# OpenDrift/opendrift

Hardware: AMD Instinct MI355X
Metric: particle-steps/sec (RK4, 3D interp) (higher is better)
Workload: dtype f64; 1 GPU; C3: OceanDrift 3D, synthetic ROMS-shaped z-level grid 1024x1024x12 (u,v,w,K), RK4 + vertical_mixing(60 s) + vertical_advection; particles_per_gpu=10000000, particles_total=10000000, stage_math=fast, spin_up_steps=200, block_every=0, inputs=resident in HBM, parallelism=particle-sharded x1, field block broadcast once per time level

## Files before the change

### include/odrift.h

```cpp
#ifndef ODRIFT_H
#define ODRIFT_H
#include <stdint.h>

#ifdef __cplusplus
extern "C" {
#endif

typedef struct odr_ctx odr_ctx;
typedef struct odr_particles odr_particles;

typedef enum {
  ODR_OK = 0,
  ODR_ERR_INVALID = -1,
  ODR_ERR_HIP = -2,
  ODR_ERR_CAPACITY = -3,
  ODR_ERR_STATE = -4
} odr_status;

enum {
  ODR_VAR_X_SEA_WATER_VELOCITY = 0,
  ODR_VAR_Y_SEA_WATER_VELOCITY = 1,
  ODR_VAR_X_WIND = 2,
  ODR_VAR_Y_WIND = 3,
  ODR_VAR_UPWARD_SEA_WATER_VELOCITY = 4,
// ... 262 lines not shown
int odr_scan_status(odr_ctx *ctx, odr_particles *p, int64_t *n_kept, uint64_t *status_flags);
int odr_scan_status_begin(odr_ctx *ctx, odr_particles *p);
int odr_scan_status_end(odr_ctx *ctx, odr_particles *p, int64_t *n_kept, uint64_t *status_flags);
int odr_ctx_guard_next_vmix(odr_ctx *ctx, int on);
int odr_compact_apply(odr_ctx *ctx, odr_particles *p, int64_t *n_active);
int odr_sort_particles(odr_ctx *ctx, odr_particles *p, int32_t source_id);
int odr_sort_particles_ex(odr_ctx *ctx, odr_particles *p, int32_t source_id, int keep_environment);
int odr_particles_tile_stats(odr_ctx *ctx, odr_particles *p, uint64_t *out4);
int odr_particles_step_layout_stats(odr_ctx *ctx, odr_particles *p, uint64_t *out2);
int odr_particles_step_onlevel_stats(odr_ctx *ctx, odr_particles *p, uint64_t *out1);
int odr_particles_vmix_layout_stats(odr_ctx *ctx, odr_particles *p, uint64_t *out3);
int odr_particles_vmix_kplane_stats(odr_ctx *ctx, odr_particles *p, uint64_t *out2);
int odr_particles_vmix_window_stats(odr_ctx *ctx, odr_particles *p, uint64_t *out3);
int odr_particles_vmix_skip_stats(odr_ctx *ctx, odr_particles *p, uint64_t *out2);
int odr_particles_vmix_dense_stats(odr_ctx *ctx, odr_particles *p, uint64_t *out2);
int odr_reduce_scalars(odr_ctx *ctx, odr_particles *p, double wind_drift_depth, double *out16);
int odr_ctx_set_step_reduce(odr_ctx *ctx, int on, double wind_drift_depth, int relative_wind);
int odr_reduce_local(odr_ctx *ctx, odr_particles *p, double wind_drift_depth, int relative_wind, double *out16);
int odr_reduce_install(odr_ctx *ctx, odr_particles *p, const double *in16);
int odr_reduce_unpin(odr_ctx *ctx);
int odr_reduce_cached(odr_ctx *ctx, odr_particles *p, double *out16, int32_t *state);

int odr_ctx_set_position_class(odr_ctx *ctx, int f32);
int odr_source_set_coordinate_dtype(odr_ctx *ctx, int32_t source_id, int x_is_float32, int y_is_float32);

#define ODR_COMM_ID_BYTES 256
int odr_device_count(int32_t *n);
int odr_comm_unique_id(uint8_t *id );
int odr_comm_init(odr_ctx *ctx, const uint8_t *id, int32_t rank, int32_t nranks);
int odr_comm_info(int32_t *rank, int32_t *nranks, uint64_t *id_hash, int32_t *rccl_version, uint64_t *collectives);
// ... 116 lines not shown
```

### opendrift_amd/_abi.py

```python
import ctypes as C
import os

HERE = os.path.dirname(os.path.abspath(__file__))
LIB_PATH = os.environ.get('ODR_LIB') or os.path.join(HERE, 'libodrift_hip.so')

NVAR = 26
VARIABLES = {
    'x_sea_water_velocity': 0, 'y_sea_water_velocity': 1, 'x_wind': 2, 'y_wind': 3,
    'upward_sea_water_velocity': 4, 'ocean_vertical_diffusivity': 5,
    'sea_surface_wave_stokes_drift_x_velocity': 6, 'sea_surface_wave_stokes_drift_y_velocity': 7,
    'land_binary_mask': 8, 'sea_floor_depth_below_sea_level': 9, 'sea_surface_height': 10,
    'horizontal_diffusivity': 11, 'sea_surface_wave_significant_height': 12,
    'sea_surface_wave_period_at_variance_spectral_density_maximum': 13,
    'ocean_mixed_layer_thickness': 14,
    'sea_water_temperature': 15, 'sea_water_salinity': 16,
    'sea_ice_area_fraction': 17, 'sea_ice_x_velocity': 18, 'sea_ice_y_velocity': 19,
    'sea_surface_swell_wave_to_direction': 20,
    'sea_surface_swell_wave_peak_period_from_variance_spectral_density': 21,
    'sea_surface_swell_wave_significant_height': 22, 'sea_surface_wind_wave_to_direction': 23,
    'sea_surface_wind_wave_mean_period': 24, 'sea_surface_wind_wave_significant_height': 25,
}
VARIABLE_NAMES = {v: k for k, v in VARIABLES.items()}
PROJ_LATLONG, PROJ_STERE_EQUIT_SPHERE, PROJ_STERE_POLAR = 0, 1, 2
PROJ_MERC, PROJ_LCC = 4, 5
# ... 168 lines not shown
    'odr_scan_status': [_vp, _vp, _i64p, _P(C.c_uint64)],
    'odr_scan_status_begin': [_vp, _vp],
    'odr_scan_status_end': [_vp, _vp, _i64p, _P(C.c_uint64)],
    'odr_ctx_guard_next_vmix': [_vp, C.c_int],
    'odr_compact_apply': [_vp, _vp, _i64p],
    'odr_sort_particles': [_vp, _vp, C.c_int32],
    'odr_sort_particles_ex': [_vp, _vp, C.c_int32, C.c_int],
    'odr_particles_tile_stats': [_vp, _vp, _P(C.c_uint64)],
    'odr_particles_step_layout_stats': [_vp, _vp, _P(C.c_uint64)],
    'odr_particles_step_onlevel_stats': [_vp, _vp, _P(C.c_uint64)],
    'odr_particles_vmix_layout_stats': [_vp, _vp, _P(C.c_uint64)],
    'odr_particles_vmix_kplane_stats': [_vp, _vp, _P(C.c_uint64)],
    'odr_particles_vmix_window_stats': [_vp, _vp, _P(C.c_uint64)],
    'odr_particles_vmix_skip_stats': [_vp, _vp, _P(C.c_uint64)],
    'odr_particles_vmix_dense_stats': [_vp, _vp, _P(C.c_uint64)],
    'odr_reduce_scalars': [_vp, _vp, C.c_double, _dp],
    'odr_ctx_set_step_reduce': [_vp, C.c_int, C.c_double, C.c_int],
    'odr_reduce_local': [_vp, _vp, C.c_double, C.c_int, _dp],
    'odr_reduce_install': [_vp, _vp, _dp],
    'odr_reduce_unpin': [_vp],
    'odr_reduce_cached': [_vp, _vp, _dp, _ip],
    'odr_timer_begin': [_vp],
    'odr_timer_end': [_vp, _fp],
    'odr_sgrid_create': [_vp, C.c_int32, C.c_int32, C.c_int32, _dp, _dp, C.c_double, _dp, _dp, C.c_int32, _P(_vp)],
    'odr_sgrid_destroy': [_vp, _vp],
    'odr_sgrid_download_zrho': [_vp, _vp, _dp],
    'odr_sgrid_zslice': [_vp, _vp, _vp, C.c_int, C.c_int, C.c_int32, _dp, C.c_int32, _P(_vp), _dp],
    'odr_history_create': [_vp, C.c_int64, C.c_int32, C.c_int32, _ip, _P(_vp)],
    'odr_history_destroy': [_vp, _vp],
    'odr_history_set_id_base': [_vp, _vp, C.c_int64],
# ... 90 lines not shown
```

### opendrift_amd/csrc/odr_host.h

```cpp
#pragma once
#include <hip/hip_runtime.h>

#include <algorithm>
#include <cmath>
#include <cstdarg>
#include <cstdio>
#include <cstdlib>
#include <cstring>
#include <initializer_list>
#include <string>
#include <vector>

#include "../../include/odrift.h"
#include "odr_kernels.hip.h"

using namespace odr;

#include <chrono>
struct SlowSpan {
  const char *what;
  std::chrono::steady_clock::time_point t0;
  static double limit() { static const double v = getenv("ODR_SLOW_CALLS") ? atof(getenv("ODR_SLOW_CALLS")) : 0.0; return v; }
  explicit SlowSpan(const char *w) : what(w) { if (limit() > 0) t0 = std::chrono::steady_clock::now(); }
  ~SlowSpan() {
// ... 118 lines not shown
  long long scan_kept;
  float env_cval[NVAR];
  long long env_cn[NVAR];
  bool env_cok[NVAR];
  bool external;
  unsigned *wg_tab, *wg_list;
  unsigned long long *wg_total, *wg_stats;
  long long wg_cap, wg_grid, wg_n, wg_list_cap;
  unsigned long long wg_launches;
  unsigned long long step_launches[3];
  unsigned long long vmix_launches[3];
  unsigned long long vmix_kplane[2];
  unsigned long long vmix_window[2];
  unsigned long long vmix_tiled;
  unsigned long long vmix_dense;
  unsigned long long *vmix_redone;
  unsigned long long *vmix_mask;
  unsigned *vmix_toff, *vmix_list;
  double *z_keep;
  long long z_keep_n;
  bool z_truncated;
  int wg_sid;
  bool wg_valid;
  unsigned wg_src_gen;
};

static inline unsigned nblk(long long n) { return (unsigned)((n + BLOCK - 1) / BLOCK); }

static inline PView view(const odr_particles *p) {
  PView v;
  v.n = p->n;
  v.lon = p->d64[0]; v.lat = p->d64[1]; v.z = p->d64[2]; v.plon = p->d64[3]; v.plat = p->d64[4];
  v.slon = p->d64[5]; v.slat = p->d64[6];
// ... 187 lines not shown
```

### opendrift_amd/csrc/odr_kernels.hip.h

```cpp
#pragma once
#include <hip/hip_runtime.h>
#include <rocrand/rocrand_kernel.h>
#include "odr_field.hip.h"

namespace odr {

#ifndef ODR_BLOCK
#define ODR_BLOCK 256
#endif
constexpr int BLOCK = ODR_BLOCK;
#ifndef ODR_POLAR_WAVES
#define ODR_POLAR_WAVES 3
#endif
#ifndef ODR_POLAR_STEP_WAVES
#define ODR_POLAR_STEP_WAVES 2
#endif
#define ODR_STEP_WAVES(PROJ) ((PROJ) == PROJ_LATLONG ? ODR_LATLONG_WAVES : ((PROJ) == PROJ_EXT ? 1 : ODR_POLAR_STEP_WAVES))
#ifndef ODR_LATLONG_WAVES
#define ODR_LATLONG_WAVES 1
#endif
#define ODR_WAVES(PROJ) ((PROJ) == PROJ_LATLONG ? ODR_LATLONG_WAVES : ((PROJ) == PROJ_EXT ? 1 : ODR_POLAR_WAVES))

__device__ __forceinline__ unsigned pid_wg_of(unsigned nb) {
  const unsigned b = blockIdx.x, per = nb >> 3, rem = nb & 7u, x = b & 7u, j = b >> 3;
// ... 833 lines not shown
  int coast_action, stranded_code, seeded_code, land_slot;
  int store_previous, geo_slot_uv;
  int seafloor, depth_slot;
  float age_dt, max_age;
  int retired_code, missing_code;
  int nmiss_grp, nmiss_rest;
  int miss_grp[4], miss_rest[4];
  int main_noise;
  int ssh_slot;
  int red_on, red_rel;
  int red_hd, red_sx, red_xw, red_pad;
  double red_wdd, red_iwdd;
  double *red;
  unsigned *wcount;
  unsigned long long *sflags;
};

#ifndef ODR_PARK_WAVES
#define ODR_PARK_WAVES 4
#endif
#ifndef ODR_PARK_WAVES_FAST3D
#define ODR_PARK_WAVES_FAST3D 5
#endif
#define ODR_PARK_WAVES_OF(PROJ, IS3D, SM) (((PROJ) == PROJ_LATLONG && (IS3D) && (SM) == 1) ? ODR_PARK_WAVES_FAST3D : ODR_PARK_WAVES)
#define ODR_STEP_PARKS(SCHEME, PROJ) ((SCHEME) > 0 && ((PROJ) == PROJ_LATLONG || (PROJ) == PROJ_CURVILINEAR))
template <int SCHEME, int PROJ, bool IS3D, bool NOISE, int SM = 0, class LY = LayoutRT>
__global__ __launch_bounds__(BLOCK, ODR_STEP_PARKS(SCHEME, PROJ) ? ODR_PARK_WAVES_OF(PROJ, IS3D, SM) : ODR_STEP_WAVES(PROJ)) void k_step_grid(const DevWorld *__restrict__ W, PView p, EnvGroupDesc G,
                                                     StepDesc S, double dt, float factor, UVTime th, UVTime tf,
                                                     unsigned long long *n_hit, StageNoise N) {
  long long i = pid();
// ... 89 lines not shown
          ps0.ok = 0;
          p.env[VAR_LAND][i] = 0.0f;
        }
      }
    }
    if (S.seafloor) {
      float floorz;
      if constexpr (LY::STATIC) {
        static_assert(LY::depth_slot >= 0 && LY::ssh_slot < 0, "a static layout holds the depth and not the ssh");
        floorz = -__fadd_rn(out[LY::depth_slot], ssh0);
      } else {
        const float dep = S.depth_slot == 2 ? out[2] : (S.depth_slot == 3 ? out[3] : p.env[VAR_DEPTH][i]);
        floorz = -__fadd_rn(dep, S.ssh_slot >= 0 ? pick_slot(out, S.ssh_slot) : ssh0);
      }
      if (zz < (double)floorz) { zz = (double)floorz; p.z[i] = zz; }
    }
    if (S.age_dt != 0.0f) {
      const float a = __fadd_rn(age0, S.age_dt);
      p.age[i] = a;
      if (S.max_age > 0 && a >= S.max_age) {
        if (st == 0) p.status[i] = st = S.retired_code;
        p.moving[i] = moving = 0;
      }
    }
    const bool skip = st != 0;
    if constexpr (IS3D && SM == 1) { if (zz != z) K.valid = false; }
    if (S.store_previous) { p.plon[i] = lon; p.plat[i] = lat; }
    ODR_PT(3);
    if (!skip) {
      const DevSource &s = W->src[G.sid];
// ... 842 lines not shown
      if (esc != 0ull) {
        if (escaped) {
          long long i2 = i;
          asm volatile("" : "+v"(i2));
          const VMixState S2 = vmix_load_state(p, i2);
          vmix_col_particle<NQ, TL, typename VM::Full>(s, p, Dp, A, vadv, i, Kp, gsh, t, S2);
          if (D.redone && (t & 63) == __ffsll((long long)esc) - 1) atomicAdd(D.redone, (unsigned long long)__popcll(esc));
        }
      }
    }
  }
}

struct VMixKeep {
  unsigned long long *mask;
  unsigned *toff;
  unsigned *list;
  unsigned *hdr;
  unsigned long long *listed;
};
__global__ __launch_bounds__(BLOCK) void k_vmix_keep(PView p, VMixKeep K, const unsigned long long *guard, double dt,
                                                      double dt_mix_cfg) {
  if (guard && *guard == 0ull) return;
  constexpr int NW = BLOCK / 64;
  __shared__ unsigned cnt[NW];
  const int tid = threadIdx.x, lane = tid & 63, wave = tid >> 6;
  const long long base = (long long)blockIdx.x * VMIX_TILE;
  double z[VMIX_TILE_ROUNDS];
  float dep[VMIX_TILE_ROUNDS], ssh[VMIX_TILE_ROUNDS];
#pragma unroll
  for (int r = 0; r < VMIX_TILE_ROUNDS; ++r) {
    const long long e = base + r * BLOCK + tid, ec = e < p.n ? e : 0;
    z[r] = p.z[ec]; dep[r] = p.env[VAR_DEPTH][ec]; ssh[r] = p.env[VAR_SSH][ec];
  }
  const double sgn = dt > 0 ? 1.0 : (dt < 0 ? -1.0 : 0.0);
  const bool walks = abs((int)(dt / (dt_mix_cfg * sgn))) > 0;
  unsigned mine = 0;
#pragma unroll
  for (int r = 0; r < VMIX_TILE_ROUNDS; ++r) {
    const long long e = base + r * BLOCK + tid;
    const float Zmin = __fmul_rn(-1.f, __fadd_rn(dep[r], ssh[r]));
    const bool skip = e < p.n && z[r] == 0 && !(Zmin > 0.f);
    if (skip && walks && __double_as_longlong(z[r]) != 0ll) p.z[e] = 0.0;
    const unsigned long long keep = __ballot(e < p.n && !skip);
    if (lane == 0) K.mask[(size_t)blockIdx.x * (VMIX_TILE / 64) + r * NW + wave] = keep;
    mine += (unsigned)__popcll(keep);
  }
  if (lane == 0) cnt[wave] = mine;
  __syncthreads();
  if (tid == 0) {
    unsigned t = 0;
#pragma unroll
    for (int w = 0; w < NW; ++w) t += cnt[w];
    K.toff[blockIdx.x] = t;
  }
}
constexpr int VMIX_SCAN_ROWS = 16;
__global__ __launch_bounds__(1024) void k_vmix_keep_scan(VMixKeep K, long long ntiles, long long n,
                                                          const unsigned long long *guard, unsigned long long *skipped) {
  const int tid = threadIdx.x, lane = tid & 63, wv = tid >> 6;
  if (guard && *guard == 0ull) {
    if (tid == 0) { K.hdr[0] = 0u; K.hdr[1] = 0u; }
    return;
  }
  constexpr int G = VMIX_SCAN_ROWS;
  __shared__ unsigned wtot[G * 16];
  unsigned carry = 0;
  for (long long k0 = 0; k0 < ntiles; k0 += (long long)G * 1024) {
    unsigned v[G], x[G];
#pragma unroll
    for (int u = 0; u < G; ++u) {
      const long long k = k0 + (long long)u * 1024 + tid;
      v[u] = k < ntiles ? K.toff[k] : 0u;
    }
#pragma unroll
    for (int u = 0; u < G; ++u) {
      x[u] = v[u];
#pragma unroll
      for (int o = 1; o < 64; o <<= 1) { const unsigned y = __shfl_up(x[u], o, 64); if (lane >= o) x[u] += y; }
      if (lane == 63) wtot[u * 16 + wv] = x[u];
    }
    __syncthreads();
    if (wv == 0) {
#pragma unroll
      for (int b0 = 0; b0 < G * 16; b0 += 64) {
        const unsigned t0 = wtot[b0 + lane];
        unsigned s = t0;
#pragma unroll
        for (int o = 1; o < 64; o <<= 1) { const unsigned y = __shfl_up(s, o, 64); if (lane >= o) s += y; }
        wtot[b0 + lane] = carry + s - t0;
        carry += __shfl(s, 63, 64);
      }
    }
    __syncthreads();
#pragma unroll
    for (int u = 0; u < G; ++u) {
      const long long k = k0 + (long long)u * 1024 + tid;
      if (k < ntiles) K.toff[k] = x[u] - v[u] + wtot[u * 16 + wv];
    }
    __syncthreads();
  }
  if (tid == 0) {
    K.hdr[0] = carry;
    K.hdr[1] = (carry + (unsigned)BLOCK - 1u) / (unsigned)BLOCK;
    if (skipped && (unsigned long long)n > carry) atomicAdd(skipped, (unsigned long long)n - carry);
    if (carry) atomicAdd(K.listed, (unsigned long long)carry);
  }
}
__global__ __launch_bounds__(BLOCK) void k_vmix_keep_fill(VMixKeep K, const unsigned long long *guard) {
  if (guard && *guard == 0ull) return;
  constexpr int NW = BLOCK / 64;
  const int tid = threadIdx.x, lane = tid & 63;
  const int wave = __builtin_amdgcn_readfirstlane(tid >> 6);
  const unsigned long long *m = K.mask + (size_t)blockIdx.x * (VMIX_TILE / 64);
  unsigned run = K.toff[blockIdx.x], off[VMIX_TILE_ROUNDS];
  unsigned long long keep[VMIX_TILE_ROUNDS];
#pragma unroll
  for (int g = 0; g < VMIX_TILE / 64; ++g) {
    const unsigned long long mg = m[g];
    if ((g % NW) == wave) { off[g / NW] = run; keep[g / NW] = mg; }
    run += (unsigned)__popcll(mg);
  }
  const unsigned long long below = (1ull << lane) - 1ull;
  const unsigned first = (unsigned)blockIdx.x * (unsigned)VMIX_TILE;
#pragma unroll
  for (int r = 0; r < VMIX_TILE_ROUNDS; ++r)
    if ((keep[r] >> lane) & 1ull) K.list[off[r] + (unsigned)__popcll(keep[r] & below)] = first + (unsigned)(r * BLOCK + tid);
}
__host__ __device__ constexpr size_t vmix_dense_lds_bytes(int nq) {
  return sizeof(double) * ((size_t)(4 * nq) * BLOCK + 4 * (size_t)(4 * nq));
}
template <int NQ, bool TL, class VM>
__global__ __launch_bounds__(BLOCK, ODR_VMIX_WAVES) void k_vmix_dense(const DevWorld *__restrict__ W, PView p, VMixDesc D,
                                                      const unsigned *__restrict__ list, const unsigned *__restrict__ hdr,
                                                      double dt, double dt_mix_cfg, int mix_at_surface,
                                                      int rng_mode, const double *__restrict__ huni,
                                                      unsigned long long seed, unsigned long long step,
                                                      int vadv, int sfl) {
  static_assert(VM::STATIC, "the dense launch exists for the static configurations");
  constexpr int NL = 4 * NQ;
  extern __shared__ __attribute__((aligned(16))) char smem[];
  const int tid = threadIdx.x;
  const DevSource &s = W->src[D.sid];
  const int nzp = VM::nzp(D.nzp, NL);
  double *Kp = (double *)smem;
  double *gsh = Kp + (size_t)NL * BLOCK;
  if (D.guard && *D.guard == 0ull) return;
  const unsigned total = hdr[0], nbd = hdr[1];
  if (blockIdx.x >= nbd) return;
  const unsigned d = pid_wg_of(nbd) * BLOCK + (unsigned)tid;
  const bool valid = d < total;
  const long long i = list[valid ? d : 0u];
  if (tid < nzp) {
    gsh[tid] = s.vg_a[tid]; gsh[NL + tid] = s.vg_b[tid]; gsh[2 * NL + tid] = s.vg_c[tid];
    gsh[3 * NL + tid] = s.zmid[tid];
  }
  long long i1 = i;
  asm volatile("" : "+v"(i1));
  const VMixState S = vmix_load_state(p, i1);
  __syncthreads();
  if (!valid) return;
  VMixArgs A;
  A.dt = dt; A.dt_mix_cfg = dt_mix_cfg; A.mix_at_surface = mix_at_surface; A.rng_mode = rng_mode; A.sfl = sfl; A.pad = 0;
  A.huni = huni; A.seed = seed; A.step = step;
  const bool escaped = vmix_col_particle<NQ, TL, VM>(s, p, D, A, vadv, i, Kp, gsh, tid, S);
  if constexpr (VM::WINDOW) {
    const unsigned long long esc = __ballot(escaped);
// ... 1481 lines not shown
```

### opendrift_amd/csrc/odr_mix.hip

```cpp
#define ODR_TU_MIX 1
#include "odr_host.h"

static_assert(vmix_col_lds_bytes(3) <= 163840 / ODR_VMIX_WAVES, "k_vmix_col<3>: column, tables and offset list exceed a sixth of the LDS");
static_assert(vmix_dense_lds_bytes(3) <= 163840 / ODR_VMIX_WAVES, "k_vmix_dense<3>: column and tables exceed a sixth of the LDS");
static_assert(VMIX_TILE == 1024, "odr_particles_create sizes the keep ballots and tile counts for tiles of 1024 elements");

template <class VM>
static bool vmix_layout_matches(const DevSource &s, const VMixDesc &D, int nq, double dt, double dt_mix, int mix_at_surface,
                                int rng_mode, int sfl, int vadv) {
  const bool uz = s.vg_uniform != 0;
  const int ntimes = abs((int)(dt / (dt_mix * (dt > 0 ? 1.0 : (dt < 0 ? -1.0 : 0.0)))));
  return VM::proj_kind(s.proj.kind) == s.proj.kind && VM::lon_mode(s.lon_mode) == s.lon_mode &&
         VM::mod360_x(s.mod360_x) == s.mod360_x && VM::nzp(D.nzp, 4 * nq) == D.nzp && VM::uniform_z(uz) == uz &&
         VM::rng_mode(rng_mode) == rng_mode && VM::mix_at_surface(mix_at_surface) == mix_at_surface &&
         VM::sf_action(sfl & 255) == (sfl & 255) && VM::vadv(vadv) == vadv && VM::ntimes(ntimes) == ntimes &&
         VM::kstride(D.kstride, nq) == D.kstride;
}

int odr_vmix(odr_ctx *c, odr_particles *p, double t, double dt, double dt_mix, int mix_at_surface, int rng_mode,
             const double *huni, uint64_t step) {
  const bool guarded = c->guard_next_vmix != 0;
  c->guard_next_vmix = 0;
  const bool oil = c->oil_owner == p;
  const bool f32prof = p->profiles_f32;
  const int cut = c->vmix_levels;
  VMixDesc D;
  bool kplanes = !getenv("ODR_NO_KPLANE");
  const bool fast = !oil && !f32prof && cut <= 0 && !getenv("ODR_NO_FAST_PATH") && build_vmix_desc(c, t, D, kplanes);
  if (guarded && (rng_mode == ODR_RNG_HOST || !fast)) return 1;
  const int vadv = c->fuse_vadv;
  c->fuse_vadv = -1;
  c->oil_owner = nullptr;
  c->vmix_levels = 0;
  c->guarded_vmix = nullptr;
  p->status_epoch++;
  p->epoch++;
  REQUIRE(dt_mix > 0 && dt != 0, "bad time steps");
  if (!p->env[VAR_DEPTH]) return fail(ODR_ERR_STATE, "sea_floor_depth_below_sea_level has not been sampled");
  if (int rs = seafloor_species_slot_ok(c, p)) return rs;
  int rc = ensure_env(c, p, VAR_SSH);
  if (rc) return rc;
  if ((rc = flush_world(c))) return rc;
  if (p->n == 0) return 0;
  int nzp = 1;
  for (int k = 0; k < c->hw.nlist[VAR_KZ]; ++k) {
    const DevSource &s = c->hw.src[c->hw.list[VAR_KZ][k]];
    if (s.kind == SRC_GRID) { nzp = s.nz > 1 ? s.nz : 1; break; }
  }
  double *du = nullptr;
// ... 32 lines not shown
    const bool spec = !win && (nq == 2 || nq == 3) &&
                      vmix_layout_matches<VMixC3Rec>(c->hw.src[D.sid], D, nq, dt, dt_mix, mix_at_surface, rng_mode, c->seafloor, vadv) &&
                      !getenv("ODR_NO_VMIX_SPEC");
    const bool specp = spec && vmix_layout_matches<VMixC3>(c->hw.src[D.sid], D, nq, dt, dt_mix, mix_at_surface, rng_mode, c->seafloor, vadv);
    const bool quadwin = spec && nq == 3 && !getenv("ODR_NO_VMIX_WINDOW");
    p->vmix_launches[win ? 2 : spec ? 1 : 0]++;
    p->vmix_kplane[kplanes ? 0 : 1]++;
    if (spec && nq == 3) p->vmix_window[quadwin ? 0 : 1]++;
    D.redone = quadwin ? p->vmix_redone : nullptr;
    D.skipped = p->vmix_redone + 1;
    D.noskip = getenv("ODR_NO_VMIX_SKIP") ? 1 : 0;
    if (!win) { g = dim3((unsigned)((p->n + VMIX_TILE - 1) / VMIX_TILE)); p->vmix_tiled++; }
    const bool dense = spec && mix_at_surface == 0 && vadv != 1 && !D.noskip && !getenv("ODR_NO_VMIX_DENSE") &&
                       p->n <= 0xffffffffLL;
    VMixKeep K;
    K.mask = p->vmix_mask; K.toff = p->vmix_toff; K.list = p->vmix_list;
    K.hdr = (unsigned *)(p->vmix_redone + 3); K.listed = p->vmix_redone + 2;
    if (dense) {
      hipLaunchKernelGGL(k_vmix_keep, g, b, 0, c->stream, v, K, D.guard, dt, dt_mix);
      hipLaunchKernelGGL(k_vmix_keep_scan, dim3(1), dim3(1024), 0, c->stream, K, (long long)g.x, (long long)p->n, D.guard, D.skipped);
      hipLaunchKernelGGL(k_vmix_keep_fill, g, b, 0, c->stream, K, D.guard);
      g = dim3(nblk(p->n));
      p->vmix_dense++;
    }
#define VMIX_DENSE(NQ, VM)                                                                                        \
  do {                                                                                                            \
    const size_t l2 = vmix_dense_lds_bytes(NQ);                                                                   \
    if (tl) hipLaunchKernelGGL((k_vmix_dense<NQ, true, VM>), g, b, l2, c->stream, c->dw, v, D, K.list, K.hdr, dt, dt_mix, \
                               mix_at_surface, rng_mode, du, c->seed, st, vadv, c->seafloor);                     \
    else hipLaunchKernelGGL((k_vmix_dense<NQ, false, VM>), g, b, l2, c->stream, c->dw, v, D, K.list, K.hdr, dt, dt_mix, \
                            mix_at_surface, rng_mode, du, c->seed, st, vadv, c->seafloor);                        \
  } while (0)
#define VMIX_COL(NQ, VM)                                                                                          \
  do {                                                                                                            \
    const size_t l2 = vmix_col_lds_bytes(NQ);                                                                     \
    if (tl) hipLaunchKernelGGL((k_vmix_col<NQ, true, VM>), g, b, l2, c->stream, c->dw, v, D, dt, dt_mix,          \
// ... 60 lines not shown
  D2H(&skipped, p->vmix_redone + 1, sizeof skipped);
  HIPCHK(hipStreamSynchronize(c->stream));
  out2[0] = p->vmix_tiled; out2[1] = skipped;
  return 0;
}

int odr_particles_vmix_dense_stats(odr_ctx *c, odr_particles *p, uint64_t *out2) {
  REQUIRE(c && p && out2, "NULL argument");
  unsigned long long listed = 0;
  D2H(&listed, p->vmix_redone + 2, sizeof listed);
  HIPCHK(hipStreamSynchronize(c->stream));
  out2[0] = p->vmix_dense; out2[1] = listed;
  return 0;
}

int odr_particles_vmix_window_stats(odr_ctx *c, odr_particles *p, uint64_t *out3) {
  REQUIRE(c && p && out3, "NULL argument");
  unsigned long long redone = 0;
  D2H(&redone, p->vmix_redone, sizeof redone);
  HIPCHK(hipStreamSynchronize(c->stream));
  out3[0] = p->vmix_window[0]; out3[1] = p->vmix_window[1]; out3[2] = redone;
  return 0;
}

int odr_vmix_set_profile_levels(odr_ctx *c, int32_t n) {
  REQUIRE(n == 0 || (n >= 2 && n <= 255), "bad level count %d", n);
  c->vmix_levels = n;
  return 0;
}

// ... 176 lines not shown
```

### opendrift_amd/csrc/odr_step.hip

```cpp
#define ODR_TU_STEP 1
#include <chrono>
#include "odr_step_launch.h"

int odr_advect_set_noise(odr_ctx *c, odr_particles *p, double std_normal, double std_uniform, int rng_mode,
                         const double *host_main, const double *host_stage, int nstage, uint64_t step) {
  c->noise_owner = nullptr;
  REQUIRE(std_normal >= 0 && std_uniform >= 0, "uncertainties must not be negative");
  REQUIRE(rng_mode == ODR_RNG_DEVICE || rng_mode == ODR_RNG_HOST, "bad rng mode");
  if (!(std_normal > 0) && !(std_uniform > 0)) return 0;
  StageNoise &N = c->noise;
  memset(&N, 0, sizeof N);
  N.on = 1; N.rng_mode = rng_mode; N.std_n = std_normal; N.std_u = std_uniform;
  N.ncomp = 2 * ((std_normal > 0) + (std_uniform > 0));
  N.seed = c->seed; N.step = (unsigned long long)step;
  if (rng_mode == ODR_RNG_HOST && p->n > 0) {
    REQUIRE(nstage >= 0 && nstage <= 3 && (nstage == 0 || host_stage), "host draws of the stage calls required in ODR_RNG_HOST mode");
    const size_t per = (size_t)N.ncomp * (size_t)p->n, need = per * (size_t)(nstage + (host_main ? 1 : 0));
    if (c->noise_buf_n < need) {
      HIPCHK(hipStreamSynchronize(c->stream));
      if (c->noise_buf) HIPCHK(hipFree(c->noise_buf));
      HIPCHK(hipMalloc((void **)&c->noise_buf, sizeof(double) * need));
      c->noise_buf_n = need;
    }
    double *d = c->noise_buf;
// ... 188 lines not shown
      const int a = slot_of(vx), b = slot_of(vy);
      if (a >= 0 && b == a + 1) { out = a; return true; }
      if (a == -1 && b == -1) { out = -1; return true; }
      if (a == -2 || b == -2) { out = -2; return a < 0 && b < 0; }
      return false;
    };
    S.red_hd = slot_of(VAR_HDIFF);
    red_in_launch = pair_of(VAR_SX, VAR_SY, S.red_sx) && pair_of(VAR_XWIND, VAR_YWIND, S.red_xw) && (S.red_xw == -2 || p->f32[0]);
    if (red_in_launch) {
      S.red_on = 1; S.red_rel = c->step_reduce_rel; S.red_wdd = c->step_reduce_wdd;
      S.red_iwdd = c->step_reduce_wdd != 0 ? 1.0 / fabs(c->step_reduce_wdd) : 0.0;
      if ((rc = odr_i_red_records(c, p, &S.red))) return rc;
    }
  }
  if (count_in_launch) { S.wcount = p->wcount; S.sflags = c->counter + 2; }
  if (N.on && (scheme > 0 || main_noise)) {
    if (scheme > 0 && N.rng_mode == ODR_RNG_HOST && !N.stage) return fail(ODR_ERR_INVALID, "no host draws for the Runge-Kutta stage calls");
    if (N.sm == ODR_STAGE_FAST && scheme > 0) odr_i_step_fast_noise(c, p, G, S, scheme, t, dt, factor, N);
    else odr_i_step_noise(c, p, G, S, scheme, t, dt, factor, N);
  } else if (N.sm == ODR_STAGE_FAST && scheme > 0) odr_i_step_fast(c, p, G, S, scheme, t, dt, factor, N);
  else step_dispatch<false>(c, p, G, S, scheme, t, dt, factor, N);
  HIPCHK(hipGetLastError());
  if (red_in_launch) {
    if ((rc = odr_i_red_finish(c, p))) return rc;
    c->red_owner = p; c->red_epoch = p->epoch; c->red_wdd = c->step_reduce_wdd; c->red_rel = c->step_reduce_rel;
    c->red_extents = false; c->red_partial = true;
  }
  mark(3);
  if (count_in_launch) { p->wcount_epoch = p->status_epoch; p->wcount_n = p->n; }
  if ((rc = coast_action ? read_counter(c, n_on_land) : 0)) return rc;
// ... 15 lines not shown
```

### opendrift_amd/csrc/odr_step_launch.h

```cpp
#pragma once
#include "odr_host.h"

template <int SCHEME, bool NOISE, int SM = 0>
static void launch_advect_grid(odr_ctx *c, odr_particles *p, int sid, double t, double dt, double factor, const StageNoise &N) {
  const DevSource &s = c->hw.src[sid];
  UVTime th = uv_time(s, t + dt / 2), tf = uv_time(s, t + dt);
  int geo = s.level_slot[0];
  bool is3d = s.slot[geo].var_nz[VAR_U] > 1;
  dim3 g(nblk(p->n)), b(BLOCK);
  PView v = view(p);
  float f = (float)factor;
#define ODR_LAUNCH(PROJ, D3) hipLaunchKernelGGL((k_advect_grid<SCHEME, PROJ, D3, NOISE, SM>), g, b, 0, c->stream, c->dw, sid, geo, v, dt, f, th, tf, N)
  switch (odr_proj_template(s.proj)) {
    case PROJ_LATLONG: if (is3d) ODR_LAUNCH(PROJ_LATLONG, true); else ODR_LAUNCH(PROJ_LATLONG, false); break;
    case PROJ_STERE_POLAR: if (is3d) ODR_LAUNCH(PROJ_STERE_POLAR, true); else ODR_LAUNCH(PROJ_STERE_POLAR, false); break;
    case PROJ_CURVILINEAR: if (is3d) ODR_LAUNCH(PROJ_CURVILINEAR, true); else ODR_LAUNCH(PROJ_CURVILINEAR, false); break;
    case PROJ_EXT: if (is3d) ODR_LAUNCH(PROJ_EXT, true); else ODR_LAUNCH(PROJ_EXT, false); break;
    default: if (is3d) ODR_LAUNCH(PROJ_STERE_EQUIT_SPHERE, true); else ODR_LAUNCH(PROJ_STERE_EQUIT_SPHERE, false); break;
  }
#undef ODR_LAUNCH
}

template <bool NOISE, int SM = 0>
static bool advect_dispatch(odr_ctx *c, odr_particles *p, int scheme, double t, double dt, double factor, const StageNoise &N) {
// ... 49 lines not shown
                             double factor, const StageNoise &N) {
  const EnvGroupDesc G = env_bind_out(G0, view(p));
  const DevSource &s = c->hw.src[G.sid];
  UVTime th = uv_time(s, t + dt / 2), tf = uv_time(s, t + dt);
  S.geo_slot_uv = s.level_slot[0];
  bool is3d = s.slot[S.geo_slot_uv].var_nz[VAR_U] > 1;
  dim3 g(nblk(p->n)), b(BLOCK);
  PView v = view(p);
  float f = (float)factor;
  if constexpr (SCHEME == 2 && !NOISE && SM == 1) {
    if (odr_proj_template(s.proj) == PROJ_LATLONG && is3d && !getenv("ODR_NO_LAYOUT_SPEC")) {
      if (layout_matches<LayoutC3>(G, S)) {
        hipLaunchKernelGGL((k_step_grid<SCHEME, PROJ_LATLONG, true, NOISE, SM, LayoutC3>), g, b, 0, c->stream, c->dw, v, G, S,
                           dt, f, th, tf, c->counter, N);
        p->step_launches[1]++;
        return;
      }
      if (layout_matches_onlevel(s, G, S, t, dt, th)) {
        hipLaunchKernelGGL((k_step_grid<SCHEME, PROJ_LATLONG, true, NOISE, SM, LayoutC3L1>), g, b, 0, c->stream, c->dw, v, G, S,
                           dt, f, th, tf, c->counter, N);
        p->step_launches[0]++;
        p->step_launches[2]++;
        return;
      }
    }
  }
  p->step_launches[0]++;
#define ODR_LAUNCH(PROJ, D3) hipLaunchKernelGGL((k_step_grid<SCHEME, PROJ, D3, NOISE, SM>), g, b, 0, c->stream, c->dw, v, G, S, dt, f, th, tf, c->counter, N)
  switch (odr_proj_template(s.proj)) {
    case PROJ_LATLONG: if (is3d) ODR_LAUNCH(PROJ_LATLONG, true); else ODR_LAUNCH(PROJ_LATLONG, false); break;
    case PROJ_STERE_POLAR: if (is3d) ODR_LAUNCH(PROJ_STERE_POLAR, true); else ODR_LAUNCH(PROJ_STERE_POLAR, false); break;
    case PROJ_CURVILINEAR: if (is3d) ODR_LAUNCH(PROJ_CURVILINEAR, true); else ODR_LAUNCH(PROJ_CURVILINEAR, false); break;
    case PROJ_EXT: if (is3d) ODR_LAUNCH(PROJ_EXT, true); else ODR_LAUNCH(PROJ_EXT, false); break;
    default: if (is3d) ODR_LAUNCH(PROJ_STERE_EQUIT_SPHERE, true); else ODR_LAUNCH(PROJ_STERE_EQUIT_SPHERE, false); break;
  }
#undef ODR_LAUNCH
}

template <bool NOISE, int SM = 0>
static void step_dispatch(odr_ctx *c, odr_particles *p, const EnvGroupDesc &G, const StepDesc &S, int scheme, double t, double dt,
                          double factor, const StageNoise &N) {
// ... 36 lines not shown
```

### opendrift_amd/csrc/odrift.hip

```cpp
#define ODR_TU_MISC 1
#include "odr_host.h"
#include "odr_mesh.h"

static thread_local std::string g_err;
int odr_i_fail(int code, const char *fmt, ...) {
  char buf[512];
  va_list ap;
  va_start(ap, fmt);
  vsnprintf(buf, sizeof buf, fmt, ap);
  va_end(ap);
  g_err = buf;
  return code;
}

const char *odr_last_error(void) { return g_err.c_str(); }
#define ODR_STR2(x) #x
#define ODR_STR(x) ODR_STR2(x)
const char *odr_version(void) { return "odrift-hip 0.2 (gfx950; mixing stream Philox4x32-" ODR_STR(ODR_MIX_ROUNDS) ")"; }

int odr_ctx_create(int device, uint64_t seed, odr_ctx **out) {
  REQUIRE(out, "out is NULL");
  HIPCHK(hipSetDevice(device));
  odr_ctx *c = new odr_ctx();
  c->device = device;
// ... 87 lines not shown

int odr_particles_create(odr_ctx *c, int64_t capacity, odr_particles **out) {
  REQUIRE(capacity > 0 && out, "capacity must be positive");
  HIPCHK(hipSetDevice(c->device));
  odr_particles *p = new odr_particles();
  memset(p, 0, sizeof(*p));
  p->cap = capacity;
  p->dead_cap = capacity;
  p->scan_kept = -1;
  for (int k = 0; k < 7; ++k) HIPCHK(hipMalloc((void **)&p->d64[k], sizeof(double) * (size_t)capacity));
  for (int k = 0; k < 3; ++k) HIPCHK(hipMalloc((void **)&p->i32[k], sizeof(int) * (size_t)capacity));
  for (int k = 0; k < 4; ++k) HIPCHK(hipMalloc((void **)&p->f32[k], sizeof(float) * (size_t)capacity));
  HIPCHK(hipMalloc((void **)&p->bcount, sizeof(unsigned) * (size_t)(nblk(capacity) + 1)));
  HIPCHK(hipMalloc((void **)&p->wcount, sizeof(unsigned) * (size_t)(nblk(capacity) + 1) * (BLOCK / 64)));
  p->wcount_epoch = ~0ull;
  HIPCHK(hipMalloc((void **)&p->vmix_redone, 4 * sizeof(unsigned long long)));
  HIPCHK(hipMemset(p->vmix_redone, 0, 4 * sizeof(unsigned long long)));
  const size_t vtiles = ((size_t)capacity + 1023) / 1024;
  HIPCHK(hipMalloc((void **)&p->vmix_mask, sizeof(unsigned long long) * 16 * vtiles));
  HIPCHK(hipMalloc((void **)&p->vmix_toff, sizeof(unsigned) * vtiles));
  HIPCHK(hipMalloc((void **)&p->vmix_list, sizeof(unsigned) * (size_t)capacity));
  *out = p;
  return 0;
}

int odr_particles_destroy(odr_ctx *c, odr_particles *p) {
  if (c->red_owner == p) c->red_owner = nullptr;
  if (c->noise_owner == p) c->noise_owner = nullptr;
  if (c->guarded_vmix == p) c->guarded_vmix = nullptr;
  if (!p) return 0;
  (void)hipStreamSynchronize(c->stream);
  auto fr = [](void *q) { if (q) (void)hipFree(q); };
  for (int k = 0; k < 7; ++k) { fr(p->d64[k]); fr(p->alt64[k]); }
  for (int k = 0; k < 3; ++k) { fr(p->i32[k]); fr(p->alti32[k]); fr(p->dead64[k]); }
  for (int k = 0; k < 4; ++k) { fr(p->f32[k]); fr(p->altf32[k]); }
  for (int k = 0; k < 2; ++k) fr(p->deadi32[k]);
  for (int k = 0; k < NVAR; ++k) { fr(p->env[k]); fr(p->altenv[k]); }
  for (int k = 0; k < 9; ++k) { fr(p->aux[k]); fr(p->altaux[k]); fr(p->aux_snap[k]); }
  fr(p->bcount);
  fr(p->wcount);
  fr(p->vmix_redone);
  fr(p->vmix_mask); fr(p->vmix_toff); fr(p->vmix_list);
  fr(p->scratch);
  fr(p->rank); fr(p->rank_words); fr(p->rank_before); fr(p->rank_bsum);
  fr(p->wg_tab); fr(p->wg_total); fr(p->wg_list); fr(p->z_keep);
  delete p;
  return 0;
}

template <class T>
static int put(odr_ctx *c, T *dst, const T *src, long long n, T dflt) {
  if (src) {
    H2D(dst, src, sizeof(T) * (size_t)n);
  } else {
    std::vector<T> tmp((size_t)n, dflt);
    H2D(dst, tmp.data(), sizeof(T) * (size_t)n);
    HIPCHK(hipStreamSynchronize(c->stream));
// ... 2093 lines not shown
    }
    const unsigned nt1 = (unsigned)ntiles + 1;
    hipLaunchKernelGGL(k_wg_count, dim3((nt1 + BLOCK - 1) / BLOCK), dim3(BLOCK), 0, c->stream, hist, ntiles, 64u * (unsigned)zb, wg_nw);
    hipLaunchKernelGGL(k_cmp_scan, dim3(1), dim3(1024), 0, c->stream, wg_nw, (long long)nt1, p->wg_total);
    hipLaunchKernelGGL(k_wg_fill, dim3((nt1 + BLOCK - 1) / BLOCK), dim3(BLOCK), 0, c->stream, hist, ntiles, 64u * (unsigned)zb, wg_nw, p->wg_tab, (unsigned)cap);
    p->wg_grid = cap; p->wg_n = p->n; p->wg_sid = sid; p->wg_src_gen = c->src_gen[sid]; p->wg_valid = true;
  }
  hipLaunchKernelGGL(k_gather_perm, dim3(nblk(p->n)), dim3(BLOCK), 0, c->stream, perm, p->n, A);
  HIPCHK(hipGetLastError());
  swap_sets(p, with_env);
  for (int v = 0; v < NVAR; ++v) {
    if (with_env) p->env_cn[v] = std::min(p->env_cn[v], p->n);
    else if (!(p->env_cok[v] && p->env_cn[v] >= p->n)) p->env_cok[v] = false;
  }
  p->status_epoch++;
  return 0;
}

struct odr_history {
  long long ntraj;
  int ntimes, nvars, stride;
  int codes[HIST_MAXV];
  float *buf;
  float *stage;
  size_t stage_floats;
  float *host;
  size_t host_floats;
  int flush_nt;
  hipStream_t copy_stream;
  hipEvent_t recorded, flushed;
// ... 307 lines not shown
```

### opendrift_amd/device.py

```python
import ctypes as C
import os

import numpy as np

from . import _abi
from ._abi import VARIABLES, check

_dp, _fp, _ip = C.POINTER(C.c_double), C.POINTER(C.c_float), C.POINTER(C.c_int32)


def _vid(v, aliases=None):
    if isinstance(v, (int, np.integer)):
        return v
    if v in VARIABLES:
        return VARIABLES[v]
    if aliases and v in aliases:
        return aliases[v]
    raise KeyError(v)


def _d(a, n=None):
    if a is None:
        return None, None
    a = np.ascontiguousarray(np.broadcast_to(np.asarray(a, dtype=np.float64), (n,)) if n is not None
# ... 1197 lines not shown
        check(self.lib.odr_particles_vmix_window_stats(self.ctx.h, self.h, out))
        return dict(windowed=int(out[0]), full=int(out[1]), redone=int(out[2]))

    def vmix_skip_stats(self):
        import ctypes as C
        out = (C.c_uint64 * 2)()
        check(self.lib.odr_particles_vmix_skip_stats(self.ctx.h, self.h, out))
        return dict(launches=int(out[0]), skipped=int(out[1]))

    def vmix_dense_stats(self):
        import ctypes as C
        out = (C.c_uint64 * 2)()
        check(self.lib.odr_particles_vmix_dense_stats(self.ctx.h, self.h, out))
        return dict(launches=int(out[0]), listed=int(out[1]))

    def reduce_global(self, combine, wind_drift_depth=0.1, relative_wind=False):
        raw = np.empty(16)
        check(self.lib.odr_reduce_local(self.ctx.h, self.h, float(wind_drift_depth), int(relative_wind), raw.ctypes.data_as(_dp)))
        g = np.ascontiguousarray(combine(raw), dtype=np.float64)
        check(self.lib.odr_reduce_install(self.ctx.h, self.h, g.ctypes.data_as(_dp)))
        return g

    def reduce_local(self, wind_drift_depth=0.1, relative_wind=False):
        raw = np.empty(16)
        check(self.lib.odr_reduce_local(self.ctx.h, self.h, float(wind_drift_depth), int(relative_wind), raw.ctypes.data_as(_dp)))
        return raw

    def reduce_install(self, combined16):
        g = np.ascontiguousarray(combined16, dtype=np.float64)
        check(self.lib.odr_reduce_install(self.ctx.h, self.h, g.ctypes.data_as(_dp)))
# ... 359 lines not shown
```

Measured before the change: 12.14 billion particle-steps/s.

## Fuse vertical-mixing keep-mask build into step kernel and skip identity list

The 3D step kernel now writes the per-wave vertical-mixing keep ballots and counts directly after the seafloor clamp, so the separate k_vmix_keep pass over particle z can be skipped when the step ran on the same epoch and particle count. The scan reads packed per-wave byte counts with SAD instructions instead of per-tile totals, and it flags the case where every particle is kept. In that case the fill kernel exits early and the dense mixing kernel indexes particles directly instead of going through the list. The cost is extra ballots and stores in the step kernel and epoch bookkeeping that must stay consistent with sorting and compaction.

```diff
diff --git a/include/odrift.h b/include/odrift.h
--- a/include/odrift.h
+++ b/include/odrift.h
@@ -300,6 +300,7 @@
 int odr_particles_vmix_window_stats(odr_ctx *ctx, odr_particles *p, uint64_t *out3);
 int odr_particles_vmix_skip_stats(odr_ctx *ctx, odr_particles *p, uint64_t *out2);
 int odr_particles_vmix_dense_stats(odr_ctx *ctx, odr_particles *p, uint64_t *out2);
+int odr_particles_vmix_keep_stats(odr_ctx *ctx, odr_particles *p, uint64_t *out3);
 int odr_reduce_scalars(odr_ctx *ctx, odr_particles *p, double wind_drift_depth, double *out16);
 int odr_ctx_set_step_reduce(odr_ctx *ctx, int on, double wind_drift_depth, int relative_wind);
 int odr_reduce_local(odr_ctx *ctx, odr_particles *p, double wind_drift_depth, int relative_wind, double *out16);
diff --git a/opendrift_amd/_abi.py b/opendrift_amd/_abi.py
--- a/opendrift_amd/_abi.py
+++ b/opendrift_amd/_abi.py
@@ -206,6 +206,7 @@
     'odr_particles_vmix_window_stats': [_vp, _vp, _P(C.c_uint64)],
     'odr_particles_vmix_skip_stats': [_vp, _vp, _P(C.c_uint64)],
     'odr_particles_vmix_dense_stats': [_vp, _vp, _P(C.c_uint64)],
+    'odr_particles_vmix_keep_stats': [_vp, _vp, _P(C.c_uint64)],
     'odr_reduce_scalars': [_vp, _vp, C.c_double, _dp],
     'odr_ctx_set_step_reduce': [_vp, C.c_int, C.c_double, C.c_int],
     'odr_reduce_local': [_vp, _vp, C.c_double, C.c_int, _dp],
diff --git a/opendrift_amd/csrc/odr_host.h b/opendrift_amd/csrc/odr_host.h
--- a/opendrift_amd/csrc/odr_host.h
+++ b/opendrift_amd/csrc/odr_host.h
@@ -156,9 +156,13 @@
   unsigned long long vmix_window[2];
   unsigned long long vmix_tiled;
   unsigned long long vmix_dense;
+  unsigned long long vmix_keep_src[2];
   unsigned long long *vmix_redone;
   unsigned long long *vmix_mask;
+  unsigned char *vmix_wcnt;
   unsigned *vmix_toff, *vmix_list;
+  unsigned long long keep_epoch;
+  long long keep_n;
   double *z_keep;
   long long z_keep_n;
   bool z_truncated;
diff --git a/opendrift_amd/csrc/odr_kernels.hip.h b/opendrift_amd/csrc/odr_kernels.hip.h
--- a/opendrift_amd/csrc/odr_kernels.hip.h
+++ b/opendrift_amd/csrc/odr_kernels.hip.h
@@ -871,6 +871,8 @@
   double *red;
   unsigned *wcount;
   unsigned long long *sflags;
+  unsigned long long *keep;
+  unsigned char *keepc;
 };
 
 #ifndef ODR_PARK_WAVES
@@ -990,6 +992,16 @@
         floorz = -__fadd_rn(dep, S.ssh_slot >= 0 ? pick_slot(out, S.ssh_slot) : ssh0);
       }
       if (zz < (double)floorz) { zz = (double)floorz; p.z[i] = zz; }
+      if constexpr (LY::STATIC && IS3D) {
+        if (S.keep) {
+          const bool at_top = zz == 0 && !(floorz > 0.f);
+          const unsigned long long kb = __ballot(!at_top), nz = __ballot(at_top && __double_as_longlong(zz) != 0ll);
+          if ((threadIdx.x & 63) == 0) {
+            S.keep[i >> 6] = kb;
+            S.keepc[i >> 6] = (unsigned char)((unsigned)__popcll(kb) | (nz ? 128u : 0u));
+          }
+        }
+      }
     }
     if (S.age_dt != 0.0f) {
       const float a = __fadd_rn(age0, S.age_dt);
@@ -1862,16 +1874,17 @@
 
 struct VMixKeep {
   unsigned long long *mask;
+  unsigned char *wcnt;
   unsigned *toff;
   unsigned *list;
   unsigned *hdr;
   unsigned long long *listed;
+  unsigned long long *idents;
 };
 __global__ __launch_bounds__(BLOCK) void k_vmix_keep(PView p, VMixKeep K, const unsigned long long *guard, double dt,
                                                       double dt_mix_cfg) {
   if (guard && *guard == 0ull) return;
   constexpr int NW = BLOCK / 64;
-  __shared__ unsigned cnt[NW];
   const int tid = threadIdx.x, lane = tid & 63, wave = tid >> 6;
   const long long base = (long long)blockIdx.x * VMIX_TILE;
   double z[VMIX_TILE_ROUNDS];
@@ -1883,7 +1896,6 @@
   }
   const double sgn = dt > 0 ? 1.0 : (dt < 0 ? -1.0 : 0.0);
   const bool walks = abs((int)(dt / (dt_mix_cfg * sgn))) > 0;
-  unsigned mine = 0;
 #pragma unroll
   for (int r = 0; r < VMIX_TILE_ROUNDS; ++r) {
     const long long e = base + r * BLOCK + tid;
@@ -1891,41 +1903,58 @@
     const bool skip = e < p.n && z[r] == 0 && !(Zmin > 0.f);
     if (skip && walks && __double_as_longlong(z[r]) != 0ll) p.z[e] = 0.0;
     const unsigned long long keep = __ballot(e < p.n && !skip);
-    if (lane == 0) K.mask[(size_t)blockIdx.x * (VMIX_TILE / 64) + r * NW + wave] = keep;
-    mine += (unsigned)__popcll(keep);
-  }
-  if (lane == 0) cnt[wave] = mine;
-  __syncthreads();
-  if (tid == 0) {
-    unsigned t = 0;
-#pragma unroll
-    for (int w = 0; w < NW; ++w) t += cnt[w];
-    K.toff[blockIdx.x] = t;
+    if (lane == 0) {
+      const size_t g = (size_t)blockIdx.x * (VMIX_TILE / 64) + r * NW + wave;
+      K.mask[g] = keep; K.wcnt[g] = (unsigned char)__popcll(keep);
+    }
   }
 }
 constexpr int VMIX_SCAN_ROWS = 16;
+__device__ __forceinline__ unsigned vmix_tile_count(uint4 q) {
+  const unsigned m = 0x7f7f7f7fu;
+  return __builtin_amdgcn_sad_u8(q.x & m, 0u, __builtin_amdgcn_sad_u8(q.y & m, 0u, __builtin_amdgcn_sad_u8(q.z & m, 0u,
+         __builtin_amdgcn_sad_u8(q.w & m, 0u, 0u))));
+}
 __global__ __launch_bounds__(1024) void k_vmix_keep_scan(VMixKeep K, long long ntiles, long long n,
                                                           const unsigned long long *guard, unsigned long long *skipped) {
   const int tid = threadIdx.x, lane = tid & 63, wv = tid >> 6;
   if (guard && *guard == 0ull) {
-    if (tid == 0) { K.hdr[0] = 0u; K.hdr[1] = 0u; }
+    if (tid == 0) { K.hdr[0] = 0u; K.hdr[1] = 0u; K.hdr[2] = 0u; }
     return;
   }
   constexpr int G = VMIX_SCAN_ROWS;
   __shared__ unsigned wtot[G * 16];
+  const int last_waves = (int)(((n + 63) >> 6) - (ntiles - 1) * (VMIX_TILE / 64));
   unsigned carry = 0;
   for (long long k0 = 0; k0 < ntiles; k0 += (long long)G * 1024) {
     unsigned v[G], x[G];
+    uint4 q[G];
 #pragma unroll
     for (int u = 0; u < G; ++u) {
       const long long k = k0 + (long long)u * 1024 + tid;
-      v[u] = k < ntiles ? K.toff[k] : 0u;
+      q[u] = k < ntiles ? ((const uint4 *)K.wcnt)[k] : make_uint4(0u, 0u, 0u, 0u);
+    }
+#pragma unroll
+    for (int u = 0; u < G; ++u) {
+      const long long k = k0 + (long long)u * 1024 + tid;
+      if (k == ntiles - 1 && last_waves < VMIX_TILE / 64) {
+        unsigned w[4] = {q[u].x, q[u].y, q[u].z, q[u].w};
+#pragma unroll
+        for (int j = 0; j < 4; ++j) {
+          const int m = last_waves - 4 * j;
+          w[j] = m >= 4 ? w[j] : (m <= 0 ? 0u : (w[j] & ((1u << (8 * m)) - 1u)));
+        }
+        q[u] = make_uint4(w[0], w[1], w[2], w[3]);
+      }
+      v[u] = vmix_tile_count(q[u]);
     }
 #pragma unroll
     for (int u = 0; u < G; ++u) {
       x[u] = v[u];
-#pragma unroll
-      for (int o = 1; o < 64; o <<= 1) { const unsigned y = __shfl_up(x[u], o, 64); if (lane >= o) x[u] += y; }
+      if (k0 + (long long)u * 1024 < ntiles) {
+#pragma unroll
+        for (int o = 1; o < 64; o <<= 1) { const unsigned y = __shfl_up(x[u], o, 64); if (lane >= o) x[u] += y; }
+      }
       if (lane == 63) wtot[u * 16 + wv] = x[u];
     }
     __syncthreads();
@@ -1949,31 +1978,50 @@
     __syncthreads();
   }
   if (tid == 0) {
+    const bool ident = (unsigned long long)n == carry;
     K.hdr[0] = carry;
     K.hdr[1] = (carry + (unsigned)BLOCK - 1u) / (unsigned)BLOCK;
+    K.hdr[2] = ident ? 1u : 0u;
     if (skipped && (unsigned long long)n > carry) atomicAdd(skipped, (unsigned long long)n - carry);
     if (carry) atomicAdd(K.listed, (unsigned long long)carry);
-  }
-}
-__global__ __launch_bounds__(BLOCK) void k_vmix_keep_fill(VMixKeep K, const unsigned long long *guard) {
+    if (ident) atomicAdd(K.idents, 1ull);
+  }
+}
+__global__ __launch_bounds__(BLOCK) void k_vmix_keep_fill(VMixKeep K, const unsigned long long *guard, long long n, double *z,
+                                                           int walks) {
   if (guard && *guard == 0ull) return;
   constexpr int NW = BLOCK / 64;
   const int tid = threadIdx.x, lane = tid & 63;
   const int wave = __builtin_amdgcn_readfirstlane(tid >> 6);
   const unsigned long long *m = K.mask + (size_t)blockIdx.x * (VMIX_TILE / 64);
+  const unsigned every = K.hdr[2];
   unsigned run = K.toff[blockIdx.x], off[VMIX_TILE_ROUNDS];
+  const uint4 cw = ((const uint4 *)K.wcnt)[blockIdx.x];
+  unsigned long long mg[VMIX_TILE / 64];
+#pragma unroll
+  for (int g = 0; g < VMIX_TILE / 64; ++g) mg[g] = m[g];
+  asm volatile("" ::"s"(every), "s"(run), "s"(cw.x), "s"(mg[0]), "s"(mg[VMIX_TILE / 64 - 1]), "s"(walks));
+  if (every) return;
+  const int left = (int)(((n + 63) >> 6) - (long long)blockIdx.x * (VMIX_TILE / 64));
   unsigned long long keep[VMIX_TILE_ROUNDS];
 #pragma unroll
   for (int g = 0; g < VMIX_TILE / 64; ++g) {
-    const unsigned long long mg = m[g];
-    if ((g % NW) == wave) { off[g / NW] = run; keep[g / NW] = mg; }
-    run += (unsigned)__popcll(mg);
+    if (g >= left) mg[g] = 0ull;
+    if ((g % NW) == wave) { off[g / NW] = run; keep[g / NW] = mg[g]; }
+    run += (unsigned)__popcll(mg[g]);
   }
   const unsigned long long below = (1ull << lane) - 1ull;
   const unsigned first = (unsigned)blockIdx.x * (unsigned)VMIX_TILE;
 #pragma unroll
   for (int r = 0; r < VMIX_TILE_ROUNDS; ++r)
     if ((keep[r] >> lane) & 1ull) K.list[off[r] + (unsigned)__popcll(keep[r] & below)] = first + (unsigned)(r * BLOCK + tid);
+  if (walks && ((cw.x | cw.y | cw.z | cw.w) & 0x80808080u)) {
+#pragma unroll
+    for (int r = 0; r < VMIX_TILE_ROUNDS; ++r) {
+      const long long e = (long long)first + r * BLOCK + tid;
+      if (e < n && !((keep[r] >> lane) & 1ull) && __double_as_longlong(z[e]) != 0ll) z[e] = 0.0;
+    }
+  }
 }
 __host__ __device__ constexpr size_t vmix_dense_lds_bytes(int nq) {
   return sizeof(double) * ((size_t)(4 * nq) * BLOCK + 4 * (size_t)(4 * nq));
@@ -1998,7 +2046,8 @@
   if (blockIdx.x >= nbd) return;
   const unsigned d = pid_wg_of(nbd) * BLOCK + (unsigned)tid;
   const bool valid = d < total;
-  const long long i = list[valid ? d : 0u];
+  const unsigned dv = valid ? d : 0u;
+  const long long i = hdr[2] ? dv : list[dv];
   if (tid < nzp) {
     gsh[tid] = s.vg_a[tid]; gsh[NL + tid] = s.vg_b[tid]; gsh[2 * NL + tid] = s.vg_c[tid];
     gsh[3 * NL + tid] = s.zmid[tid];
diff --git a/opendrift_amd/csrc/odr_mix.hip b/opendrift_amd/csrc/odr_mix.hip
--- a/opendrift_amd/csrc/odr_mix.hip
+++ b/opendrift_amd/csrc/odr_mix.hip
@@ -33,6 +33,7 @@
   c->oil_owner = nullptr;
   c->vmix_levels = 0;
   c->guarded_vmix = nullptr;
+  const bool step_keep = !p->external && p->keep_epoch == p->epoch && p->keep_n == p->n;
   p->status_epoch++;
   p->epoch++;
   REQUIRE(dt_mix > 0 && dt != 0, "bad time steps");
@@ -95,12 +96,15 @@
     const bool dense = spec && mix_at_surface == 0 && vadv != 1 && !D.noskip && !getenv("ODR_NO_VMIX_DENSE") &&
                        p->n <= 0xffffffffLL;
     VMixKeep K;
-    K.mask = p->vmix_mask; K.toff = p->vmix_toff; K.list = p->vmix_list;
-    K.hdr = (unsigned *)(p->vmix_redone + 3); K.listed = p->vmix_redone + 2;
+    K.mask = p->vmix_mask; K.wcnt = p->vmix_wcnt; K.toff = p->vmix_toff; K.list = p->vmix_list;
+    K.hdr = (unsigned *)(p->vmix_redone + 3); K.listed = p->vmix_redone + 2; K.idents = p->vmix_redone + 5;
     if (dense) {
-      hipLaunchKernelGGL(k_vmix_keep, g, b, 0, c->stream, v, K, D.guard, dt, dt_mix);
+      if (!step_keep) hipLaunchKernelGGL(k_vmix_keep, g, b, 0, c->stream, v, K, D.guard, dt, dt_mix);
+      p->vmix_keep_src[step_keep ? 0 : 1]++;
       hipLaunchKernelGGL(k_vmix_keep_scan, dim3(1), dim3(1024), 0, c->stream, K, (long long)g.x, (long long)p->n, D.guard, D.skipped);
-      hipLaunchKernelGGL(k_vmix_keep_fill, g, b, 0, c->stream, K, D.guard);
+      const double sg = dt > 0 ? 1.0 : (dt < 0 ? -1.0 : 0.0);
+      const int walks = abs((int)(dt / (dt_mix * sg))) > 0 ? 1 : 0;
+      hipLaunchKernelGGL(k_vmix_keep_fill, g, b, 0, c->stream, K, D.guard, (long long)p->n, v.z, walks);
       g = dim3(nblk(p->n));
       p->vmix_dense++;
     }
@@ -191,6 +195,15 @@
   return 0;
 }
 
+int odr_particles_vmix_keep_stats(odr_ctx *c, odr_particles *p, uint64_t *out3) {
+  REQUIRE(c && p && out3, "NULL argument");
+  unsigned long long idents = 0;
+  D2H(&idents, p->vmix_redone + 5, sizeof idents);
+  HIPCHK(hipStreamSynchronize(c->stream));
+  out3[0] = p->vmix_keep_src[0]; out3[1] = p->vmix_keep_src[1]; out3[2] = idents;
+  return 0;
+}
+
 int odr_particles_vmix_window_stats(odr_ctx *c, odr_particles *p, uint64_t *out3) {
   REQUIRE(c && p && out3, "NULL argument");
   unsigned long long redone = 0;
diff --git a/opendrift_amd/csrc/odr_step.hip b/opendrift_amd/csrc/odr_step.hip
--- a/opendrift_amd/csrc/odr_step.hip
+++ b/opendrift_amd/csrc/odr_step.hip
@@ -226,6 +226,9 @@
     }
   }
   if (count_in_launch) { S.wcount = p->wcount; S.sflags = c->counter + 2; }
+  if (S.seafloor && depth_slot >= 0 && p->vmix_mask && p->vmix_wcnt && !p->external && !getenv("ODR_NO_STEP_KEEP")) {
+    S.keep = p->vmix_mask; S.keepc = p->vmix_wcnt;
+  }
   if (N.on && (scheme > 0 || main_noise)) {
     if (scheme > 0 && N.rng_mode == ODR_RNG_HOST && !N.stage) return fail(ODR_ERR_INVALID, "no host draws for the Runge-Kutta stage calls");
     if (N.sm == ODR_STAGE_FAST && scheme > 0) odr_i_step_fast_noise(c, p, G, S, scheme, t, dt, factor, N);
diff --git a/opendrift_amd/csrc/odr_step_launch.h b/opendrift_amd/csrc/odr_step_launch.h
--- a/opendrift_amd/csrc/odr_step_launch.h
+++ b/opendrift_amd/csrc/odr_step_launch.h
@@ -87,6 +87,7 @@
         hipLaunchKernelGGL((k_step_grid<SCHEME, PROJ_LATLONG, true, NOISE, SM, LayoutC3>), g, b, 0, c->stream, c->dw, v, G, S,
                            dt, f, th, tf, c->counter, N);
         p->step_launches[1]++;
+        if (S.keep) { p->keep_epoch = p->epoch; p->keep_n = p->n; }
         return;
       }
       if (layout_matches_onlevel(s, G, S, t, dt, th)) {
@@ -94,10 +95,12 @@
                            dt, f, th, tf, c->counter, N);
         p->step_launches[0]++;
         p->step_launches[2]++;
+        if (S.keep) { p->keep_epoch = p->epoch; p->keep_n = p->n; }
         return;
       }
     }
   }
+  S.keep = nullptr; S.keepc = nullptr;
   p->step_launches[0]++;
 #define ODR_LAUNCH(PROJ, D3) hipLaunchKernelGGL((k_step_grid<SCHEME, PROJ, D3, NOISE, SM>), g, b, 0, c->stream, c->dw, v, G, S, dt, f, th, tf, c->counter, N)
   switch (odr_proj_template(s.proj)) {
diff --git a/opendrift_amd/csrc/odrift.hip b/opendrift_amd/csrc/odrift.hip
--- a/opendrift_amd/csrc/odrift.hip
+++ b/opendrift_amd/csrc/odrift.hip
@@ -125,10 +125,12 @@
   HIPCHK(hipMalloc((void **)&p->bcount, sizeof(unsigned) * (size_t)(nblk(capacity) + 1)));
   HIPCHK(hipMalloc((void **)&p->wcount, sizeof(unsigned) * (size_t)(nblk(capacity) + 1) * (BLOCK / 64)));
   p->wcount_epoch = ~0ull;
-  HIPCHK(hipMalloc((void **)&p->vmix_redone, 4 * sizeof(unsigned long long)));
-  HIPCHK(hipMemset(p->vmix_redone, 0, 4 * sizeof(unsigned long long)));
+  HIPCHK(hipMalloc((void **)&p->vmix_redone, 6 * sizeof(unsigned long long)));
+  HIPCHK(hipMemset(p->vmix_redone, 0, 6 * sizeof(unsigned long long)));
+  p->keep_epoch = ~0ull;
   const size_t vtiles = ((size_t)capacity + 1023) / 1024;
   HIPCHK(hipMalloc((void **)&p->vmix_mask, sizeof(unsigned long long) * 16 * vtiles));
+  HIPCHK(hipMalloc((void **)&p->vmix_wcnt, 16 * vtiles));
   HIPCHK(hipMalloc((void **)&p->vmix_toff, sizeof(unsigned) * vtiles));
   HIPCHK(hipMalloc((void **)&p->vmix_list, sizeof(unsigned) * (size_t)capacity));
   *out = p;
@@ -151,7 +153,7 @@
   fr(p->bcount);
   fr(p->wcount);
   fr(p->vmix_redone);
-  fr(p->vmix_mask); fr(p->vmix_toff); fr(p->vmix_list);
+  fr(p->vmix_mask); fr(p->vmix_wcnt); fr(p->vmix_toff); fr(p->vmix_list);
   fr(p->scratch);
   fr(p->rank); fr(p->rank_words); fr(p->rank_before); fr(p->rank_bsum);
   fr(p->wg_tab); fr(p->wg_total); fr(p->wg_list); fr(p->z_keep);
@@ -2275,6 +2277,7 @@
     else if (!(p->env_cok[v] && p->env_cn[v] >= p->n)) p->env_cok[v] = false;
   }
   p->status_epoch++;
+  p->keep_epoch = ~0ull;
   return 0;
 }
 
diff --git a/opendrift_amd/device.py b/opendrift_amd/device.py
--- a/opendrift_amd/device.py
+++ b/opendrift_amd/device.py
@@ -1235,6 +1235,12 @@
         check(self.lib.odr_particles_vmix_dense_stats(self.ctx.h, self.h, out))
         return dict(launches=int(out[0]), listed=int(out[1]))
 
+    def vmix_keep_stats(self):
+        import ctypes as C
+        out = (C.c_uint64 * 3)()
+        check(self.lib.odr_particles_vmix_keep_stats(self.ctx.h, self.h, out))
+        return dict(from_step=int(out[0]), from_keep=int(out[1]), identity=int(out[2]))
+
     def reduce_global(self, combine, wind_drift_depth=0.1, relative_wind=False):
         raw = np.empty(16)
         check(self.lib.odr_reduce_local(self.ctx.h, self.h, float(wind_drift_depth), int(relative_wind), raw.ctypes.data_as(_dp)))
```

Result: faster. 12.39 billion particle-steps/s (median of 6 runs) (+2.1%).
